# zhupan007/Detection_3D

Measured on AMD Instinct MI355X. Metric: buildings/sec inference, 4c_fpn432, higher is better.
Workload: dtype f32

## Files before the change

### detection_3d_amd/csrc/roi_align.hip

```cpp
#include <algorithm>

#include "d3d_internal.h"

namespace d3d {

struct RoiGeom {
  int b;
  float cw, ch, cz, bh, bw, bz, sh, sw, sz, cosT, sinT;
  int gh, gw, gz;
};
__device__ __forceinline__ RoiGeom roi_geom(const float *r, float spatial_scale, int PH, int PW, int PZ,
                                            int sampling_ratio) {
  RoiGeom g;
  g.b = (int)r[0];
  g.cw = r[1] * spatial_scale;
  g.ch = r[2] * spatial_scale;
  g.cz = r[3] * spatial_scale;
  float rw = r[4] * spatial_scale, rh = r[5] * spatial_scale, rz = r[6] * spatial_scale;
  const float theta = (float)((double)r[7] * 3.14159265358979323846 / 180.0);
  rw = fmaxf(rw, 1.f);
  rh = fmaxf(rh, 1.f);
  rz = fmaxf(rz, 1.f);
  g.bh = rh / (float)PH;
  g.bw = rw / (float)PW;
  g.bz = rz / (float)PZ;
  g.gh = sampling_ratio > 0 ? sampling_ratio : (int)ceilf(rh / PH);
  g.gw = sampling_ratio > 0 ? sampling_ratio : (int)ceilf(rw / PW);
  g.gz = sampling_ratio > 0 ? sampling_ratio : (int)ceilf(rz / PZ);
  g.sh = (float)(-rh / 2.0);
  g.sw = (float)(-rw / 2.0);
  g.sz = (float)(-rz / 2.0);
  g.cosT = (float)cos((double)theta);
  g.sinT = (float)sin((double)theta);
  return g;
}
__device__ __forceinline__ void sample_pos(const RoiGeom &g, int ph, int pw, int pz, int iy, int ix,
                                           int iz, float &y, float &x, float &z) {
  const float yy = g.sh + ph * g.bh + (float)(iy + .5f) * g.bh / (float)g.gh;
  const float xx = g.sw + pw * g.bw + (float)(ix + .5f) * g.bw / (float)g.gw;
  const float zz = g.sz + pz * g.bz + (float)(iz + .5f) * g.bz / (float)g.gz;
  x = xx * g.cosT + yy * g.sinT + g.cw;
  y = yy * g.cosT - xx * g.sinT + g.ch;
  z = zz + g.cz;
}
struct Tri {
  int yl, yh, xl, xh, zl, zh;
  float ly, lx, lz, hy, hx, hz;
};
__device__ __forceinline__ bool tri_setup(float y, float x, float z, int H, int W, int Z, Tri &t) {
  if (y < -1.0 || y > H || x < -1.0 || x > W || z < -1.0) return false;
  if (y <= 0) y = 0;
  if (x <= 0) x = 0;
  if (z <= 0) z = 0;
  t.yl = (int)y;
  t.xl = (int)x;
  t.zl = (int)z;
  if (t.yl >= H - 1) { t.yh = t.yl = H - 1; y = (float)t.yl; } else t.yh = t.yl + 1;
  if (t.xl >= W - 1) { t.xh = t.xl = W - 1; x = (float)t.xl; } else t.xh = t.xl + 1;
  if (t.zl >= Z - 1) { t.zh = t.zl = Z - 1; z = (float)t.zl; } else t.zh = t.zl + 1;
  t.ly = y - t.yl;
  t.lx = x - t.xl;
  t.lz = z - t.zl;
  t.hy = 1. - t.ly;
  t.hx = 1. - t.lx;
  t.hz = 1. - t.lz;
  return true;
}

__global__ __launch_bounds__(256) void k_roi_dense(const float *__restrict__ input, int C, int H,
                                                   int W, int Z, const float *__restrict__ rois,
                                                   long nthreads, float spatial_scale, int PH, int PW,
                                                   int PZ, int sampling_ratio, float *__restrict__ out) {
  long index = (long)blockIdx.x * blockDim.x + threadIdx.x;
  if (index >= nthreads) return;
  const int pz = index % PZ;
  const int pw = (index / PZ) % PW;
  const int ph = (index / PZ / PW) % PH;
  const int c = (index / PZ / PW / PH) % C;
  const int n = index / PZ / PW / PH / C;
  const RoiGeom g = roi_geom(rois + (size_t)n * 8, spatial_scale, PH, PW, PZ, sampling_ratio);
  const float *d = input + ((size_t)g.b * C + c) * H * W * Z;
  const float count = (float)(g.gh * g.gw * g.gz);
  float acc = 0.f;
  for (int iy = 0; iy < g.gh; iy++)
    for (int ix = 0; ix < g.gw; ix++)
      for (int iz = 0; iz < g.gz; iz++) {
        float y, x, z;
        sample_pos(g, ph, pw, pz, iy, ix, iz, y, x, z);
        Tri t;
        if (!tri_setup(y, x, z, H, W, Z, t)) continue;
        const float v1 = d[(t.yl * W + t.xl) * Z + t.zl], v2 = d[(t.yl * W + t.xh) * Z + t.zl];
        const float v3 = d[(t.yh * W + t.xl) * Z + t.zl], v4 = d[(t.yh * W + t.xh) * Z + t.zl];
        const float v5 = d[(t.yl * W + t.xl) * Z + t.zh], v6 = d[(t.yl * W + t.xh) * Z + t.zh];
        const float v7 = d[(t.yh * W + t.xl) * Z + t.zh], v8 = d[(t.yh * W + t.xh) * Z + t.zh];
        const float w1 = t.hy * t.hx * t.hz, w2 = t.hy * t.lx * t.hz, w3 = t.ly * t.hx * t.hz, w4 = t.ly * t.lx * t.hz;
        const float w5 = t.hy * t.hx * t.lz, w6 = t.hy * t.lx * t.lz, w7 = t.ly * t.hx * t.lz, w8 = t.ly * t.lx * t.lz;
        acc += (w1 * v1 + w2 * v2 + w3 * v3 + w4 * v4 + w5 * v5 + w6 * v6 + w7 * v7 + w8 * v8);
      }
  out[index] = acc / count;
}

static constexpr int kRoiG = 4;
static constexpr int kRoiCch = 128;
__device__ __forceinline__ void roi_wave_sync() {
  __builtin_amdgcn_fence(__ATOMIC_RELEASE, "wavefront");
  __builtin_amdgcn_wave_barrier();
  __builtin_amdgcn_fence(__ATOMIC_ACQUIRE, "wavefront");
}
static constexpr int kRoiWaves = 4;
struct RoiLevel {
  const HashEntry *tab;
  const void *feats;
  const int32_t *extent;
  const int32_t *dense;
  int cap, H, W, Z;
  int e0, e1, e2;
  float scale;
};
static constexpr int kRoiMaxLevels = 4;
struct RoiLevels {
  RoiLevel v[kRoiMaxLevels];
};
template <typename T>
__global__ __launch_bounds__(kRoiWaves * 64) __attribute__((amdgpu_waves_per_eu(4, 4))) void k_roi_sparse(
    RoiLevels lv, int C, const float *__restrict__ rois, const int32_t *__restrict__ roi_levels,
    int PH, int PW, int PZ, int sampling_ratio, int layout, T *__restrict__ out) {
  const int n = blockIdx.x, cc = blockIdx.y;
  const int l = roi_levels ? __builtin_amdgcn_readfirstlane(roi_levels[n]) : 0;
  if (l < 0 || l >= kRoiMaxLevels) return;
  RoiLevel L = lv.v[0];
  if (l == 1) L = lv.v[1];
  if (l == 2) L = lv.v[2];
  if (l == 3) L = lv.v[3];
  if (!L.tab) return;
  const HashEntry *__restrict__ tab = L.tab;
  const int32_t *__restrict__ dense = L.dense;
  const T *__restrict__ feats = (const T *)L.feats;
  const int cap = L.cap;
  const float spatial_scale = L.scale;
  int H = L.H, W = L.W, Z = L.Z;
  if (L.extent) {
    H = L.extent[0];
    W = L.extent[1];
    Z = L.extent[2];
  }
  typedef float f32x2 __attribute__((ext_vector_type(2)));
  __shared__ int2 list[kRoiWaves][kRoiG][64];
  const int NB = PH * PW * PZ;
  const int wave = threadIdx.x >> 6, lane = threadIdx.x & 63;
  const RoiGeom g = roi_geom(rois + (size_t)n * 8, spatial_scale, PH, PW, PZ, sampling_ratio);
  const int NS = g.gh * g.gw * g.gz;
  const float count = (float)NS;
  const int c0 = cc * kRoiCch + 2 * lane;
  const bool ok0 = c0 < C, ok1 = c0 + 1 < C;
  const bool pair = ok1 && (C % 2 == 0);
  const size_t n_out = (size_t)n;
  auto load2 = [&](int row) -> f32x2 {
    const T *p = feats + (size_t)row * C + c0;
    f32x2 v = {0.f, 0.f};
    if (pair) {
      if constexpr (sizeof(T) == 4) {
        v = *(const f32x2 *)p;
      } else {
        const unsigned u = *(const unsigned *)p;
        v[0] = __uint_as_float(u << 16);
        v[1] = __uint_as_float(u & 0xffff0000u);
      }
    } else {
      if (ok0) v[0] = ld1(p);
      if (ok1) v[1] = ld1(p + 1);
    }
    return v;
  };
  const int ngroups = (NB + kRoiG - 1) / kRoiG;
  for (int grp = wave; grp < ngroups; grp += kRoiWaves) {
    const int b0 = grp * kRoiG;
    f32x2 acc[kRoiG];
#pragma unroll
    for (int gi = 0; gi < kRoiG; gi++) acc[gi] = {0.f, 0.f};
    for (int s0 = 0; s0 < NS; s0 += 8) {
      const int s = s0 + (lane >> 3), corner = lane & 7;
      const int iz = s % g.gz, ix = (s / g.gz) % g.gw, iy = s / (g.gz * g.gw);
      const int zb = corner >> 2, yb = (corner >> 1) & 1, xb = corner & 1;
      int row[kRoiG];
      float wgt[kRoiG];
      static_assert(kRoiG % 4 == 0, "probe groups of four");
#pragma unroll
      for (int g0 = 0; g0 < kRoiG; g0 += 4) {
        uint64_t key[4];
        bool want[4];
        int r4[4];
#pragma unroll
        for (int j = 0; j < 4; j++) {
          const int bin = b0 + g0 + j;
          wgt[g0 + j] = 0.f;
          key[j] = 0;
          want[j] = false;
          if (s < NS && bin < NB) {
            const int pz = bin % PZ, pw = (bin / PZ) % PW, ph = bin / (PZ * PW);
            float y, x, z;
            sample_pos(g, ph, pw, pz, iy, ix, iz, y, x, z);
            Tri t;
            if (tri_setup(y, x, z, H, W, Z, t)) {
              wgt[g0 + j] = (yb ? t.ly : t.hy) * (xb ? t.lx : t.hx) * (zb ? t.lz : t.hz);
              key[j] = pack_key(g.b, yb ? t.yh : t.yl, xb ? t.xh : t.xl, zb ? t.zh : t.zl);
              want[j] = true;
            }
          }
        }
        if (dense) {
          int v4[4];
#pragma unroll
          for (int j = 0; j < 4; j++) {
            const uint64_t kk = key[j];
            const size_t cell = ((((size_t)(kk >> 48) * L.e0 + (size_t)((kk >> 32) & 0xffff)) * L.e1 +
                                  (size_t)((kk >> 16) & 0xffff)) * L.e2 + (size_t)(kk & 0xffff));
            v4[j] = want[j] ? dense[cell] : 0;
          }
#pragma unroll
          for (int j = 0; j < 4; j++) r4[j] = v4[j] - 1;
        } else {
          hash_find_n<4>(tab, cap, key, want, r4);
        }
#pragma unroll
        for (int j = 0; j < 4; j++) row[g0 + j] = r4[j];
      }
      int cnt[kRoiG];
#pragma unroll
      for (int gi = 0; gi < kRoiG; gi++) {
        unsigned long long m = __ballot(row[gi] >= 0);
        int c = 0;
        while (m) {
          const int rl = __shfl(row[gi], __builtin_ctzll(m), 64);
          const bool mine = row[gi] == rl;
          float w = mine ? wgt[gi] : 0.f;
#pragma unroll
          for (int d = 32; d >= 1; d >>= 1) w += __shfl_xor(w, d, 64);
          if (lane == 0) list[wave][gi][c] = make_int2(rl, __float_as_int(w));
          c++;
          m &= ~__ballot(mine);
        }
        cnt[gi] = c;
      }
      roi_wave_sync();
#pragma unroll
      for (int gi = 0; gi < kRoiG; gi++) {
        const int2 *L = list[wave][gi];
        const int nc = cnt[gi];
        int i = 0;
        for (; i + 8 <= nc; i += 8) {
          int2 e[8];
          f32x2 v[8];
#pragma unroll
          for (int j = 0; j < 8; j++) e[j] = L[i + j];
#pragma unroll
          for (int j = 0; j < 8; j++) v[j] = load2(e[j].x);
#pragma unroll
          for (int j = 0; j < 8; j++) acc[gi] += __int_as_float(e[j].y) * v[j];
        }
        if (i + 4 <= nc) {
          int2 e[4];
          f32x2 v[4];
#pragma unroll
          for (int j = 0; j < 4; j++) e[j] = L[i + j];
#pragma unroll
          for (int j = 0; j < 4; j++) v[j] = load2(e[j].x);
#pragma unroll
          for (int j = 0; j < 4; j++) acc[gi] += __int_as_float(e[j].y) * v[j];
          i += 4;
        }
        if (i + 2 <= nc) {
          const int2 e0 = L[i], e1 = L[i + 1];
          const f32x2 v0 = load2(e0.x), v1 = load2(e1.x);
          acc[gi] += __int_as_float(e0.y) * v0;
          acc[gi] += __int_as_float(e1.y) * v1;
          i += 2;
        }
        if (i < nc) {
          const int2 e0 = L[i];
          acc[gi] += __int_as_float(e0.y) * load2(e0.x);
        }
      }
      roi_wave_sync();
    }
#pragma unroll
    for (int gi = 0; gi < kRoiG; gi++) {
      const int bin = b0 + gi;
      if (bin >= NB) break;
      const f32x2 r = acc[gi] / count;
      if (layout == 0) {
        T *o = out + (n_out * C + c0) * NB + bin;
        if (ok0) st1(o, r[0]);
        if (ok1) st1(o + NB, r[1]);
      } else {
        const int pz = bin % PZ, cell = bin / PZ;
        T *o = out + ((n_out * (size_t)(PH * PW) + cell) * C + c0) * PZ + pz;
        if (ok0) st1(o, r[0]);
        if (ok1) st1(o + PZ, r[1]);
      }
    }
  }
}

__global__ __launch_bounds__(256) void k_roi_dense_bwd(const float *__restrict__ top_diff, int C, int H, int W,
                                                       int Z, const float *__restrict__ rois, long nthreads,
                                                       float spatial_scale, int PH, int PW, int PZ,
                                                       int sampling_ratio, float *__restrict__ bottom_diff) {
  long index = (long)blockIdx.x * blockDim.x + threadIdx.x;
  if (index >= nthreads) return;
  const int pz = index % PZ;
  const int pw = (index / PZ) % PW;
  const int ph = (index / PZ / PW) % PH;
  const int c = (index / PZ / PW / PH) % C;
  const int n = index / PZ / PW / PH / C;
  const RoiGeom g = roi_geom(rois + (size_t)n * 8, spatial_scale, PH, PW, PZ, sampling_ratio);
  float *d = bottom_diff + ((size_t)g.b * C + c) * H * W * Z;
  const float count = (float)(g.gh * g.gw * g.gz);
  const float top = top_diff[index];
  for (int iy = 0; iy < g.gh; iy++)
    for (int ix = 0; ix < g.gw; ix++)
      for (int iz = 0; iz < g.gz; iz++) {
        float y, x, z;
        sample_pos(g, ph, pw, pz, iy, ix, iz, y, x, z);
        Tri t;
        if (z > Z || !tri_setup(y, x, z, H, W, Z, t)) continue;
        const float w[8] = {t.hy * t.hx * t.hz, t.hy * t.lx * t.hz, t.ly * t.hx * t.hz, t.ly * t.lx * t.hz,
                            t.hy * t.hx * t.lz, t.hy * t.lx * t.lz, t.ly * t.hx * t.lz, t.ly * t.lx * t.lz};
#pragma unroll
        for (int q = 0; q < 8; q++) {
          const int yy = (q >> 1) & 1 ? t.yh : t.yl, xx = q & 1 ? t.xh : t.xl, zz = q >> 2 ? t.zh : t.zl;
          atomicAdd(d + ((size_t)yy * W + xx) * Z + zz, top * w[q] / count);
        }
      }
}

static constexpr int kRoiBwdCch = 64;
template <typename TT>
__global__ __launch_bounds__(256) void k_roi_sparse_bwd(
    const HashEntry *__restrict__ tab, int cap, int C, int H, int W, int Z, const float *__restrict__ rois,
    float spatial_scale, int PH, int PW, int PZ, int sampling_ratio, const TT *__restrict__ top_diff,
    float *__restrict__ d_feats) {
  extern __shared__ float tile[];
  const int n = blockIdx.x, cc = blockIdx.y;
  const int NB = PH * PW * PZ, LD = NB + 1;
  const int wave = threadIdx.x >> 6, lane = threadIdx.x & 63;
  const int nch = min(kRoiBwdCch, C - cc * kRoiBwdCch);
  const TT *g0 = top_diff + ((size_t)n * C + (size_t)cc * kRoiBwdCch) * NB;
  for (int idx = threadIdx.x; idx < nch * NB; idx += 256) tile[(idx / NB) * LD + idx % NB] = ld1(g0 + idx);
  __syncthreads();
  const RoiGeom g = roi_geom(rois + (size_t)n * 8, spatial_scale, PH, PW, PZ, sampling_ratio);
  const int NS = g.gh * g.gw * g.gz;
  const float count = (float)NS;
  const int c = cc * kRoiBwdCch + lane;
  const bool cok = c < C;
  for (int bin = wave; bin < NB; bin += 4) {
    const int pz = bin % PZ, pw = (bin / PZ) % PW, ph = bin / (PZ * PW);
    const float top = cok ? tile[lane * LD + bin] : 0.f;
    for (int s0 = 0; s0 < NS; s0 += 8) {
      const int s = s0 + (lane >> 3), corner = lane & 7;
      int row = -1;
      float wgt = 0.f;
      if (s < NS) {
        const int iz = s % g.gz, ix = (s / g.gz) % g.gw, iy = s / (g.gz * g.gw);
        float y, x, z;
        sample_pos(g, ph, pw, pz, iy, ix, iz, y, x, z);
        Tri t;
        if (!(z > Z) && tri_setup(y, x, z, H, W, Z, t)) {
          const int zb = corner >> 2, yb = (corner >> 1) & 1, xb = corner & 1;
          wgt = (yb ? t.ly : t.hy) * (xb ? t.lx : t.hx) * (zb ? t.lz : t.hz);
          row = hash_find(tab, cap, pack_key(g.b, yb ? t.yh : t.yl, xb ? t.xh : t.xl, zb ? t.zh : t.zl));
        }
      }
      unsigned long long m = __ballot(row >= 0);
      while (m) {
        const int rr = __shfl(row, __builtin_ctzll(m), 64);
        const bool mine = row == rr;
        float ww = mine ? wgt : 0.f;
#pragma unroll
        for (int d = 32; d >= 1; d >>= 1) ww += __shfl_xor(ww, d, 64);
        if (cok) atomicAdd(d_feats + (size_t)rr * C + c, top * ww / count);
        m &= ~__ballot(mine);
      }
    }
  }
}

static constexpr int kRoiDetChunk = 64;
static constexpr int kRoiDetCpl = 4;

template <typename TT>
__global__ __launch_bounds__(256) void k_roi_det_transpose(const TT *__restrict__ in, int C, int NB,
                                                           float *__restrict__ out) {
  __shared__ float t[32][33];
  const int n = blockIdx.x, b0 = blockIdx.y * 32, c0 = blockIdx.z * 32;
  const int tx = threadIdx.x & 31, ty = threadIdx.x >> 5;
  const TT *src = in + (size_t)n * C * NB;
  for (int j = ty; j < 32; j += 8) {
    const int c = c0 + j, b = b0 + tx;
    t[j][tx] = (c < C && b < NB) ? ld1(src + (size_t)c * NB + b) : 0.f;
  }
  __syncthreads();
  float *dst = out + (size_t)n * NB * C;
  for (int j = ty; j < 32; j += 8) {
    const int b = b0 + j, c = c0 + tx;
    if (c < C && b < NB) dst[(size_t)b * C + c] = t[tx][j];
  }
}

template <bool WRITE>
__global__ __launch_bounds__(256) void k_roi_det_taps(
    const HashEntry *__restrict__ tab, int cap, int H, int W, int Z, const float *__restrict__ rois,
    float spatial_scale, int PH, int PW, int PZ, int sampling_ratio, int n_rows, int32_t *__restrict__ cnt,
    const int32_t *__restrict__ offs, uint32_t *__restrict__ rec_key, int32_t *__restrict__ rec_val,
    int32_t *__restrict__ rec_src, float *__restrict__ rec_w) {
  const int n = blockIdx.x;
  const int NB = PH * PW * PZ;
  const int wave = threadIdx.x >> 6, lane = threadIdx.x & 63;
  const RoiGeom g = roi_geom(rois + (size_t)n * 8, spatial_scale, PH, PW, PZ, sampling_ratio);
  const int NS = g.gh * g.gw * g.gz;
  const float count = (float)NS;
  for (int bin = wave; bin < NB; bin += 4) {
    const int pz = bin % PZ, pw = (bin / PZ) % PW, ph = bin / (PZ * PW);
    const int src = n * NB + bin;
    int pos = WRITE ? offs[src] : 0;
    for (int s0 = 0; s0 < NS; s0 += 8) {
      const int s = s0 + (lane >> 3), corner = lane & 7;
      int row = -1;
      float wgt = 0.f;
      if (s < NS) {
        const int iz = s % g.gz, ix = (s / g.gz) % g.gw, iy = s / (g.gz * g.gw);
        float y, x, z;
        sample_pos(g, ph, pw, pz, iy, ix, iz, y, x, z);
        Tri t;
        if (!(z > Z) && tri_setup(y, x, z, H, W, Z, t)) {
          const int zb = corner >> 2, yb = (corner >> 1) & 1, xb = corner & 1;
          wgt = (yb ? t.ly : t.hy) * (xb ? t.lx : t.hx) * (zb ? t.lz : t.hz);
          row = hash_find(tab, cap, pack_key(g.b, yb ? t.yh : t.yl, xb ? t.xh : t.xl, zb ? t.zh : t.zl));
          if (row >= n_rows) row = -1;
        }
      }
      unsigned long long m = __ballot(row >= 0);
      while (m) {
        const int rr = __shfl(row, __builtin_ctzll(m), 64);
        const bool mine = row == rr;
        if (WRITE) {
          float ww = mine ? wgt : 0.f;
#pragma unroll
          for (int d = 32; d >= 1; d >>= 1) ww += __shfl_xor(ww, d, 64);
          if (lane == 0) {
            rec_key[pos] = (uint32_t)rr;
            rec_val[pos] = pos;
            rec_src[pos] = src;
            rec_w[pos] = ww / count;
          }
        }
        pos++;
        m &= ~__ballot(mine);
      }
    }
    if (!WRITE && lane == 0) cnt[src] = pos;
  }
}

__global__ __launch_bounds__(256) void k_roi_det_bounds(const uint32_t *__restrict__ skey, int n_max,
                                                        const int32_t *__restrict__ total, int32_t *__restrict__ rbeg,
                                                        int32_t *__restrict__ rend) {
  const int i = blockIdx.x * 256 + threadIdx.x;
  const int n = *total;
  if (i >= n || i >= n_max) return;
  const uint32_t k = skey[i];
  if (i == 0 || skey[i - 1] != k) rbeg[k] = i;
  if (i == n - 1 || skey[i + 1] != k) rend[k] = i + 1;
}

template <typename TO>
__global__ __launch_bounds__(256) void k_roi_det_sum(const uint32_t *__restrict__ skey, const int32_t *__restrict__ sval,
                                                     const int32_t *__restrict__ rec_src, const float *__restrict__ rec_w,
                                                     int n_max, const int32_t *__restrict__ total,
                                                     const int32_t *__restrict__ rbeg, const int32_t *__restrict__ rend,
                                                     const float *__restrict__ topT, int C, float *__restrict__ part,
                                                     TO *__restrict__ d_feats) {
  const int wave = threadIdx.x >> 6, lane = threadIdx.x & 63;
  const int chunk = blockIdx.x * 4 + wave;
  const int a = chunk * kRoiDetChunk;
  const int n = min(*total, n_max);
  if (a >= n) return;
  const int len = min(kRoiDetChunk, n - a);
  int my_key = -1, my_src = 0;
  float my_w = 0.f;
  if (lane < len) {
    my_key = (int)skey[a + lane];
    const int v = sval[a + lane];
    my_src = rec_src[v];
    my_w = rec_w[v];
  }
  for (int cb = 0; cb < C; cb += 64 * kRoiDetCpl) {
    float acc[kRoiDetCpl];
#pragma unroll
    for (int j = 0; j < kRoiDetCpl; j++) acc[j] = 0.f;
    int cur = __shfl(my_key, 0, 64), seg = 0;
    auto flush = [&](int row, int sa, int sb) {
      const bool whole = rbeg[row] == a + sa && rend[row] == a + sb;
      if (whole) {
        TO *dst = d_feats + (size_t)row * C;
#pragma unroll
        for (int j = 0; j < kRoiDetCpl; j++) {
          const int c = cb + lane + 64 * j;
          if (c < C) {
            if constexpr (sizeof(TO) == 4) dst[c] = dst[c] + acc[j];
            else st1(dst + c, acc[j]);
          }
          acc[j] = 0.f;
        }
      } else {
        float *dst = part + ((size_t)chunk * 2 + (sa == 0 ? 0 : 1)) * C;
#pragma unroll
        for (int j = 0; j < kRoiDetCpl; j++) {
          const int c = cb + lane + 64 * j;
          if (c < C) dst[c] = acc[j];
          acc[j] = 0.f;
        }
      }
    };
    for (int p0 = 0; p0 < len; p0 += 4) {
      int key[4], src[4];
      float w[4], v[4][kRoiDetCpl];
#pragma unroll
      for (int q = 0; q < 4; q++) {
        key[q] = __shfl(my_key, p0 + q, 64);
        src[q] = __shfl(my_src, p0 + q, 64);
        w[q] = __shfl(my_w, p0 + q, 64);
      }
#pragma unroll
      for (int q = 0; q < 4; q++)
#pragma unroll
        for (int j = 0; j < kRoiDetCpl; j++) {
          const int c = cb + lane + 64 * j;
          v[q][j] = (p0 + q < len && c < C) ? topT[(size_t)src[q] * C + c] : 0.f;
        }
#pragma unroll
      for (int q = 0; q < 4; q++) {
        if (p0 + q >= len) break;
        if (key[q] != cur) {
          flush(cur, seg, p0 + q);
          cur = key[q];
          seg = p0 + q;
        }
#pragma unroll
        for (int j = 0; j < kRoiDetCpl; j++) acc[j] += w[q] * v[q][j];
      }
    }
    flush(cur, seg, len);
  }
}

template <typename TO>
__global__ __launch_bounds__(256) void k_roi_det_join(const int32_t *__restrict__ rbeg, const int32_t *__restrict__ rend,
                                                      int n_rows, const float *__restrict__ part, int C,
                                                      TO *__restrict__ d_feats) {
  const int row = blockIdx.x * 4 + (threadIdx.x >> 6), lane = threadIdx.x & 63;
  if (row >= n_rows) return;
  const int rb = rbeg[row], re = rend[row];
  if (re <= rb) return;
  const int c0 = rb / kRoiDetChunk, c1 = (re - 1) / kRoiDetChunk;
  if (c0 == c1) return;
  for (int c = lane; c < C; c += 64) {
    float acc = 0.f;
    for (int k = c0; k <= c1; k++) {
      const int slot = (k == c0 && rb != k * kRoiDetChunk) ? 1 : 0;
      acc += part[((size_t)k * 2 + slot) * C + c];
    }
    if constexpr (sizeof(TO) == 4) d_feats[(size_t)row * C + c] += acc;
    else st1(d_feats + (size_t)row * C + c, acc);
  }
}

__global__ __launch_bounds__(256) void k_roi_f32_to_bf16(const float *__restrict__ in, long n,
                                                         unsigned short *__restrict__ out) {
  const long i = ((long)blockIdx.x * 256 + threadIdx.x) * 4;
  if (i + 4 <= n)
    store4(out + i, load4<float>(in + i));
  else
    for (long j = i; j < n; j++) st1(out + j, in[j]);
}

struct RoiDetLayout {
  size_t cnt, offs, total, scan, rkey, rval, rsrc, rw, skey, sval, sort, rbeg, rend, topT, part, bytes;
  size_t scan_bytes, sort_bytes;
  long n_max, n_src, n_chunks;
  int bits;
};
static bool roi_det_layout(int K, int C, int ph, int pw, int pz, int sampling_ratio, int n_rows, RoiDetLayout &L) {
  if (K < 0 || C <= 0 || ph <= 0 || pw <= 0 || pz <= 0 || sampling_ratio <= 0 || n_rows < 0) return false;
  const long NB = (long)ph * pw * pz, NS = (long)sampling_ratio * sampling_ratio * sampling_ratio;
  L.n_src = (long)K * NB;
  L.n_max = L.n_src * NS * 8;
  if (L.n_max >= (1L << 31) - kRoiDetChunk) return false;
  L.n_chunks = (L.n_max + kRoiDetChunk - 1) / kRoiDetChunk;
  L.bits = 1;
  while (L.bits < 31 && (1L << L.bits) < (long)n_rows) L.bits++;
  size_t o = 0;
  auto take = [&](size_t bytes) {
    const size_t at = o;
    o = (o + bytes + 255) & ~size_t(255);
    return at;
  };
  L.cnt = take(4 * L.n_src);
  L.offs = take(4 * L.n_src);
  L.total = take(4);
  L.scan_bytes = 4 * ((L.n_src + 2047) / 2048 + 1) + 256;
  L.scan = take(L.scan_bytes);
  L.rkey = take(4 * L.n_max);
  L.rval = take(4 * L.n_max);
  L.rsrc = take(4 * L.n_max);
  L.rw = take(4 * L.n_max);
  L.skey = take(4 * L.n_max);
  L.sval = take(4 * L.n_max);
  L.sort_bytes = sort_scratch_bytes((int)std::max(L.n_max, 1L), L.bits);
  L.sort = take(L.sort_bytes);
  L.rbeg = take(4 * (size_t)n_rows);
  L.rend = take(4 * (size_t)n_rows);
  L.topT = take(4 * (size_t)L.n_src * C);
  L.part = take(4 * (size_t)L.n_chunks * 2 * C);
  L.bytes = o + 256;
  return true;
}

static constexpr int kRoiFormFields = 13;
static thread_local int t_roi_last_form[kRoiFormFields] = {};
enum RoiFamily { kRoiFamDense = 1, kRoiFamSparse = 2, kRoiFamDenseBwd = 3, kRoiFamSparseBwd = 4, kRoiFamDet = 5 };
static void roi_record(int family, size_t type_bytes, int lookup, int extent, dim3 grid, int block, int levels, long cvt = 0,
                       long n_max = 0, long n_chunks = 0, int bits = 0) {
  const int f[kRoiFormFields] = {family, type_bytes == 4 ? 1 : 2, lookup, extent, (int)grid.x, (int)grid.y, (int)grid.z,
                                 block, levels, (int)cvt, (int)n_max, (int)n_chunks, bits};
  std::copy(f, f + kRoiFormFields, t_roi_last_form);
}
static void roi_record_sparse(const RoiLevels &lv, size_t type_bytes, dim3 grid) {
  int lookup = 0, extent = 0, levels = 0;
  for (int l = 0; l < kRoiMaxLevels; l++) {
    if (!lv.v[l].tab) continue;
    levels++;
    lookup |= lv.v[l].dense ? 2 : 1;
    extent |= lv.v[l].extent ? 2 : 1;
  }
  roi_record(kRoiFamSparse, type_bytes, lookup, extent, grid, kRoiWaves * 64, levels);
}

}

using namespace d3d;

struct RoiPrepScales {
  float v[8];
};
__global__ __launch_bounds__(256) void k_roi_prepare(const float *__restrict__ boxes, int n, float voxel_scale,
                                                     RoiPrepScales scales, int n_levels, float inv_canonical,
                                                     float *__restrict__ rois, int32_t *__restrict__ levels,
                                                     const int32_t *__restrict__ batch_ids,
                                                     const int32_t *__restrict__ count) {
  const int i = blockIdx.x * blockDim.x + threadIdx.x;
  if (i >= n) return;
  if (count && i >= *count) {
    float *r = rois + (size_t)i * 8;
#pragma unroll
    for (int j = 0; j < 8; j++) r[j] = 0.f;
    if (levels) levels[i] = -1;
    return;
  }
  float b[7];
#pragma unroll
  for (int j = 0; j < 7; j++) b[j] = boxes[(size_t)i * 7 + j];
#pragma unroll
  for (int j = 0; j < 6; j++) b[j] *= voxel_scale;
  const float kHalfPi = (float)(3.14159265358979323846 * 0.5), kPi = (float)3.14159265358979323846;
  const float kInvPi = 1.f / kPi, kDeg = (float)(180.0 / 3.14159265358979323846);
  float yaw = b[6] + kHalfPi;
  yaw = yaw - floorf(yaw * kInvPi + 0.f) * kPi;
  float *r = rois + (size_t)i * 8;
  r[0] = batch_ids ? (float)batch_ids[i] : 0.f;
  r[1] = b[1];
  r[2] = b[0];
  r[3] = b[2] + b[5] * 0.5f;
  r[4] = b[3];
  r[5] = b[4];
  r[6] = b[5];
  r[7] = yaw * kDeg;
  if (levels) {
    const float rate = sqrtf(fmaxf(b[3], b[4])) * inv_canonical;
    int best = 0;
    float bd = fabsf(scales.v[0] - rate);
    for (int l = 1; l < n_levels; l++) {
      const float d = fabsf(scales.v[l] - rate);
      if (d < bd) {
        bd = d;
        best = l;
      }
    }
    levels[i] = best;
  }
}

extern "C" {

int d3d_roi_prepare(const float *boxes_metric, int n, float voxel_scale, const float *scales_host, int n_levels,
                    float canonical_size, const int32_t *batch_ids, float *rois, int32_t *levels, void *stream) {
  return d3d_roi_prepare_counted(boxes_metric, n, nullptr, voxel_scale, scales_host, n_levels, canonical_size, batch_ids,
                                 rois, levels, stream);
}

int d3d_roi_prepare_counted(const float *boxes_metric, int n, const int32_t *count_dev, float voxel_scale,
                            const float *scales_host, int n_levels, float canonical_size, const int32_t *batch_ids,
                            float *rois, int32_t *levels, void *stream) {
  hipStream_t s = (hipStream_t)stream;
  D3D_REQUIRE(n >= 0 && n_levels >= 0 && n_levels <= 8, "roi_prepare: bad arguments (at most 8 levels)");
  if (n == 0) return D3D_OK;
  D3D_REQUIRE(boxes_metric && rois && (n_levels == 0 || scales_host), "roi_prepare: null pointer");
  RoiPrepScales sc = {};
  for (int l = 0; l < n_levels; l++) sc.v[l] = scales_host[l];
  hipLaunchKernelGGL(k_roi_prepare, dim3((unsigned)((n + 255) / 256)), dim3(256), 0, s, boxes_metric, n, voxel_scale, sc,
                     n_levels, 1.f / canonical_size, rois, n_levels > 1 ? levels : nullptr, batch_ids, count_dev);
  D3D_LAUNCH_CHECK();
  return D3D_OK;
}

int d3d_roi_align_rotated_3d_forward(const float *input, int B, int C, int H, int W, int Z,
                                     const float *rois, int K, float spatial_scale, int ph, int pw,
                                     int pz, int sampling_ratio, float *out, void *stream) {
  hipStream_t s = (hipStream_t)stream;
  D3D_REQUIRE(B > 0 && C > 0 && H > 0 && W > 0 && Z > 0 && K >= 0 && ph > 0 && pw > 0 && pz > 0, "roi_align: bad shape");
  if (K == 0) return D3D_OK;
  D3D_REQUIRE(input && rois && out, "roi_align: null pointer");
  long nthreads = (long)K * C * ph * pw * pz;
  hipLaunchKernelGGL(k_roi_dense, dim3((unsigned)((nthreads + 255) / 256)), dim3(256), 0, s, input, C, H, W, Z, rois, nthreads, spatial_scale, ph, pw, pz, sampling_ratio, out);
  D3D_LAUNCH_CHECK();
  roi_record(kRoiFamDense, 4, 0, 0, dim3((unsigned)((nthreads + 255) / 256)), 256, 0);
  return D3D_OK;
}

static int roi_level_of(d3d_meta *m, const int *size, const void *feats, const int *crop, float spatial_scale,
                        hipStream_t s, RoiLevel *lv) {
  std::map<Size3, Grid>::iterator it;
  bool have_grid;
  {
    D3D_LOCK(m);
    it = m->grids.find(Size3{size[0], size[1], size[2]});
    have_grid = it != m->grids.end();
  }
  if (!have_grid) {
    set_error("roi_align_sparse: no grid of spatial size [%d,%d,%d]", size[0], size[1], size[2]);
    return D3D_ERR_STATE;
  }
  Grid &g = it->second;
  const int32_t *extent = nullptr;
  if (!crop) {
    int rc = grid_extent(m, g, s);
    if (rc) return rc;
    extent = g.extent;
  }
  *lv = {g.tab, feats, extent, crop ? nullptr : g.dense, g.cap, crop ? crop[0] : 0, crop ? crop[1] : 0, crop ? crop[2] : 0,
         g.hext[0], g.hext[1], g.hext[2], spatial_scale};
  return D3D_OK;
}

}

template <typename T>
static int roi_sparse_forward(d3d_meta *m, const int *size, const T *feats, int C, const int *crop, const float *rois, int K,
                              float spatial_scale, int ph, int pw, int pz, int sampling_ratio, const int *roi_levels,
                              int level, int layout, T *out, void *stream) {
  hipStream_t s = (hipStream_t)stream;
  D3D_REQUIRE(m && size && C > 0 && K >= 0 && ph > 0 && pw > 0 && pz > 0, "roi_align_sparse: bad arguments");
  D3D_REQUIRE(!roi_levels || (level >= 0 && level < kRoiMaxLevels), "roi_align_sparse: level %d (< %d)", level, kRoiMaxLevels);
  D3D_REQUIRE(sizeof(T) == 4 || ((uintptr_t)feats & 3) == 0, "roi_align_sparse: bf16 rows not 4-byte aligned");
  RoiLevels lv = {};
  if (int rc = roi_level_of(m, size, feats, crop, spatial_scale, s, &lv.v[roi_levels ? level : 0])) return rc;
  if (K == 0) return D3D_OK;
  D3D_REQUIRE(feats && rois && out, "roi_align_sparse: null pointer");
  D3D_REQUIRE(layout == 0 || layout == 1, "roi_align_sparse: layout must be 0 ([K,C,ph,pw,pz]) or 1 ([K,ph,pw,C,pz])");
  hipLaunchKernelGGL(k_roi_sparse<T>, dim3(K, (C + kRoiCch - 1) / kRoiCch), dim3(kRoiWaves * 64), 0, s, lv, C, rois,
                     roi_levels, ph, pw, pz, sampling_ratio, layout, out);
  D3D_LAUNCH_CHECK();
  roi_record_sparse(lv, sizeof(T), dim3(K, (C + kRoiCch - 1) / kRoiCch));
  return D3D_OK;
}

template <typename T>
static int roi_sparse_forward_levels(d3d_meta *m, int n_levels, const int *sizes_host, const T *const *feats_host, int C,
                                     const float *scales_host, const float *rois, int K, int ph, int pw, int pz,
                                     int sampling_ratio, const int *roi_levels, int layout, T *out, void *stream) {
  hipStream_t s = (hipStream_t)stream;
  D3D_REQUIRE(m && sizes_host && feats_host && scales_host && n_levels >= 1 && n_levels <= kRoiMaxLevels,
              "roi_align_sparse_levels: 1..%d levels", kRoiMaxLevels);
  D3D_REQUIRE(C > 0 && K >= 0 && ph > 0 && pw > 0 && pz > 0 && (roi_levels || n_levels == 1),
              "roi_align_sparse_levels: bad arguments");
  D3D_REQUIRE(layout == 0 || layout == 1, "roi_align_sparse: layout must be 0 ([K,C,ph,pw,pz]) or 1 ([K,ph,pw,C,pz])");
  RoiLevels lv = {};
  for (int l = 0; l < n_levels; l++) {
    D3D_REQUIRE(feats_host[l], "roi_align_sparse_levels: null feature pointer of level %d", l);
    D3D_REQUIRE(sizeof(T) == 4 || ((uintptr_t)feats_host[l] & 3) == 0, "roi_align_sparse_levels: bf16 rows not 4-byte aligned");
    if (int rc = roi_level_of(m, sizes_host + 3 * l, feats_host[l], nullptr, scales_host[l], s, &lv.v[l])) return rc;
  }
  if (K == 0) return D3D_OK;
  D3D_REQUIRE(rois && out, "roi_align_sparse_levels: null pointer");
  hipLaunchKernelGGL(k_roi_sparse<T>, dim3(K, (C + kRoiCch - 1) / kRoiCch), dim3(kRoiWaves * 64), 0, s, lv, C, rois,
                     roi_levels, ph, pw, pz, sampling_ratio, layout, out);
  D3D_LAUNCH_CHECK();
  roi_record_sparse(lv, sizeof(T), dim3(K, (C + kRoiCch - 1) / kRoiCch));
  return D3D_OK;
}

extern "C" {

int d3d_roi_align_rotated_3d_sparse_forward(d3d_meta *m, const int *size, const float *feats, int C,
                                            const int *crop, const float *rois, int K,
                                            float spatial_scale, int ph, int pw, int pz,
                                            int sampling_ratio, const int *roi_levels, int level, int layout,
                                            float *out, void *stream) {
  return roi_sparse_forward<float>(m, size, feats, C, crop, rois, K, spatial_scale, ph, pw, pz, sampling_ratio, roi_levels,
                                   level, layout, out, stream);
}

int d3d_roi_align_rotated_3d_sparse_forward_bf16(d3d_meta *m, const int *size, const void *feats, int C, const int *crop,
                                                 const float *rois, int K, float spatial_scale, int ph, int pw, int pz,
                                                 int sampling_ratio, const int *roi_levels, int level, int layout,
                                                 void *out, void *stream) {
  return roi_sparse_forward<unsigned short>(m, size, (const unsigned short *)feats, C, crop, rois, K, spatial_scale, ph,
                                            pw, pz, sampling_ratio, roi_levels, level, layout, (unsigned short *)out,
                                            stream);
}

int d3d_roi_align_rotated_3d_sparse_forward_levels(d3d_meta *m, int n_levels, const int *sizes_host,
                                                   const float *const *feats_host, int C, const float *scales_host,
                                                   const float *rois, int K, int ph, int pw, int pz, int sampling_ratio,
                                                   const int *roi_levels, int layout, float *out, void *stream) {
  return roi_sparse_forward_levels<float>(m, n_levels, sizes_host, feats_host, C, scales_host, rois, K, ph, pw, pz,
                                          sampling_ratio, roi_levels, layout, out, stream);
}

int d3d_roi_align_rotated_3d_sparse_forward_levels_bf16(d3d_meta *m, int n_levels, const int *sizes_host,
                                                        const void *const *feats_host, int C, const float *scales_host,
                                                        const float *rois, int K, int ph, int pw, int pz,
                                                        int sampling_ratio, const int *roi_levels, int layout, void *out,
                                                        void *stream) {
  return roi_sparse_forward_levels<unsigned short>(m, n_levels, sizes_host, (const unsigned short *const *)feats_host, C,
                                                   scales_host, rois, K, ph, pw, pz, sampling_ratio, roi_levels, layout,
                                                   (unsigned short *)out, stream);
}

int d3d_roi_align_rotated_3d_backward(const float *top_diff, int B, int C, int H, int W, int Z,
                                      const float *rois, int K, float spatial_scale, int ph, int pw, int pz,
                                      int sampling_ratio, float *bottom_diff, void *stream) {
  hipStream_t s = (hipStream_t)stream;
  D3D_REQUIRE(B > 0 && C > 0 && H > 0 && W > 0 && Z > 0 && K >= 0 && ph > 0 && pw > 0 && pz > 0 && bottom_diff,
              "roi_align_backward: bad arguments");
  D3D_HIP_CHECK(hipMemsetAsync(bottom_diff, 0, sizeof(float) * (size_t)B * C * H * W * Z, s));
  if (K == 0) return D3D_OK;
  D3D_REQUIRE(top_diff && rois, "roi_align_backward: null pointer");
  long nthreads = (long)K * C * ph * pw * pz;
  hipLaunchKernelGGL(k_roi_dense_bwd, dim3((unsigned)((nthreads + 255) / 256)), dim3(256), 0, s, top_diff, C, H, W, Z,
                     rois, nthreads, spatial_scale, ph, pw, pz, sampling_ratio, bottom_diff);
  D3D_LAUNCH_CHECK();
  roi_record(kRoiFamDenseBwd, 4, 0, 0, dim3((unsigned)((nthreads + 255) / 256)), 256, 0);
  return D3D_OK;
}

static int roi_grid_of(d3d_meta *m, const int *size, const char *what, const Grid **out) {
  std::map<Size3, Grid>::iterator it;
  bool have_grid;
  {
    D3D_LOCK(m);
    it = m->grids.find(Size3{size[0], size[1], size[2]});
    have_grid = it != m->grids.end();
  }
  if (!have_grid) {
    set_error("%s: no grid of spatial size [%d,%d,%d]", what, size[0], size[1], size[2]);
    return D3D_ERR_STATE;
  }
  *out = &it->second;
  return D3D_OK;
}

int d3d_roi_align_rotated_3d_sparse_backward(d3d_meta *m, const int *size, const float *top_diff, int C,
                                             const int *crop, const float *rois, int K, float spatial_scale,
                                             int ph, int pw, int pz, int sampling_ratio, float *d_feats,
                                             void *stream) {
  hipStream_t s = (hipStream_t)stream;
  D3D_REQUIRE(m && size && crop && C > 0 && K >= 0 && ph > 0 && pw > 0 && pz > 0, "roi_align_sparse_backward: bad arguments");
  const Grid *gp;
  if (int rc = roi_grid_of(m, size, "roi_align_sparse_backward", &gp)) return rc;
  if (K == 0) return D3D_OK;
  D3D_REQUIRE(top_diff && rois && d_feats, "roi_align_sparse_backward: null pointer");
  const Grid &g = *gp;
  const int NB = ph * pw * pz;
  size_t lds = (size_t)kRoiBwdCch * (NB + 1) * sizeof(float);
  D3D_REQUIRE(lds <= 64 * 1024, "roi_align_sparse_backward: pooled volume %d too large", NB);
  hipLaunchKernelGGL(k_roi_sparse_bwd<float>, dim3(K, (C + kRoiBwdCch - 1) / kRoiBwdCch), dim3(256), lds, s, g.tab, g.cap,
                     C, crop[0], crop[1], crop[2], rois, spatial_scale, ph, pw, pz, sampling_ratio, top_diff, d_feats);
  D3D_LAUNCH_CHECK();
  roi_record(kRoiFamSparseBwd, 4, 1, 1, dim3(K, (C + kRoiBwdCch - 1) / kRoiBwdCch), 256, 1);
  return D3D_OK;
}

size_t d3d_roi_align_rotated_3d_sparse_backward_bf16_scratch_bytes(int C, int n_rows) {
  if (C <= 0 || n_rows < 0) return 0;
  return (size_t)n_rows * C * sizeof(float) + 256;
}

int d3d_roi_align_rotated_3d_sparse_backward_bf16(d3d_meta *m, const int *size, const void *top_diff, int C,
                                                  const int *crop, const float *rois, int K, float spatial_scale, int ph,
                                                  int pw, int pz, int sampling_ratio, void *d_feats, int n_rows,
                                                  void *scratch, size_t scratch_bytes, void *stream) {
  hipStream_t s = (hipStream_t)stream;
  D3D_REQUIRE(m && size && crop && C > 0 && K >= 0 && ph > 0 && pw > 0 && pz > 0 && n_rows >= 0,
              "roi_align_sparse_backward_bf16: bad arguments");
  const int NB = ph * pw * pz;
  const size_t lds = (size_t)kRoiBwdCch * (NB + 1) * sizeof(float);
  D3D_REQUIRE(lds <= 64 * 1024, "roi_align_sparse_backward_bf16: pooled volume %d too large", NB);
  const size_t need = d3d_roi_align_rotated_3d_sparse_backward_bf16_scratch_bytes(C, n_rows);
  D3D_REQUIRE(scratch_bytes >= need, "roi_align_sparse_backward_bf16: scratch %zu < %zu bytes", scratch_bytes, need);
  const Grid *gp;
  if (int rc = roi_grid_of(m, size, "roi_align_sparse_backward_bf16", &gp)) return rc;
  D3D_REQUIRE(n_rows == gp->n, "roi_align_sparse_backward_bf16: n_rows %d != %d active sites", n_rows, gp->n);
  if (n_rows == 0) return D3D_OK;
  D3D_REQUIRE(d_feats && scratch && (K == 0 || (top_diff && rois)), "roi_align_sparse_backward_bf16: null pointer");
  D3D_REQUIRE(((uintptr_t)d_feats & 7) == 0, "roi_align_sparse_backward_bf16: d_feats not 8-byte aligned");
  float *acc = (float *)(((uintptr_t)scratch + 255) & ~(uintptr_t)255);
  const long total = (long)n_rows * C;
  D3D_HIP_CHECK(hipMemsetAsync(acc, 0, sizeof(float) * (size_t)total, s));
  if (K > 0) {
    const Grid &g = *gp;
    hipLaunchKernelGGL(k_roi_sparse_bwd<unsigned short>, dim3(K, (C + kRoiBwdCch - 1) / kRoiBwdCch), dim3(256), lds, s,
                       g.tab, g.cap, C, crop[0], crop[1], crop[2], rois, spatial_scale, ph, pw, pz, sampling_ratio,
                       (const unsigned short *)top_diff, acc);
  }
  hipLaunchKernelGGL(k_roi_f32_to_bf16, dim3((unsigned)((total + 1023) / 1024)), dim3(256), 0, s, acc, total,
                     (unsigned short *)d_feats);
  D3D_LAUNCH_CHECK();
  roi_record(kRoiFamSparseBwd, 2, 1, 1, K > 0 ? dim3(K, (C + kRoiBwdCch - 1) / kRoiBwdCch) : dim3(0, 0, 0), 256, 1,
             (total + 1023) / 1024);
  return D3D_OK;
}

size_t d3d_roi_align_rotated_3d_sparse_backward_deterministic_scratch_bytes(int K, int C, int ph, int pw, int pz,
                                                                           int sampling_ratio, int n_rows) {
  RoiDetLayout L;
  return roi_det_layout(K, C, ph, pw, pz, sampling_ratio, n_rows, L) ? L.bytes : 0;
}

size_t d3d_roi_align_rotated_3d_sparse_backward_deterministic_bf16_scratch_bytes(int K, int C, int ph, int pw, int pz,
                                                                                int sampling_ratio, int n_rows) {
  return d3d_roi_align_rotated_3d_sparse_backward_deterministic_scratch_bytes(K, C, ph, pw, pz, sampling_ratio, n_rows);
}

}

template <typename TT, typename TO>
static int roi_det_run(const Grid &g, const int *crop, const TT *top_diff, int C, const float *rois, int K,
                       float spatial_scale, int ph, int pw, int pz, int sampling_ratio, TO *d_feats, int n_rows,
                       const RoiDetLayout &L, void *scratch, hipStream_t s) {
  char *base = (char *)(((uintptr_t)scratch + 255) & ~(uintptr_t)255);
  int32_t *cnt = (int32_t *)(base + L.cnt), *offs = (int32_t *)(base + L.offs), *total = (int32_t *)(base + L.total);
  uint32_t *rkey = (uint32_t *)(base + L.rkey), *skey = (uint32_t *)(base + L.skey);
  int32_t *rval = (int32_t *)(base + L.rval), *sval = (int32_t *)(base + L.sval), *rsrc = (int32_t *)(base + L.rsrc);
  float *rw = (float *)(base + L.rw), *topT = (float *)(base + L.topT), *part = (float *)(base + L.part);
  int32_t *rbeg = (int32_t *)(base + L.rbeg), *rend = (int32_t *)(base + L.rend);
  const int NB = ph * pw * pz;
  hipLaunchKernelGGL(k_roi_det_transpose<TT>, dim3(K, (NB + 31) / 32, (C + 31) / 32), dim3(256), 0, s, top_diff, C, NB,
                     topT);
  hipLaunchKernelGGL((k_roi_det_taps<false>), dim3(K), dim3(256), 0, s, g.tab, g.cap, crop[0], crop[1], crop[2], rois,
                     spatial_scale, ph, pw, pz, sampling_ratio, n_rows, cnt, nullptr, nullptr, nullptr, nullptr, nullptr);
  D3D_LAUNCH_CHECK();
  Arena scan_arena;
  scan_arena.base = base + L.scan;
  scan_arena.cap = L.scan_bytes;
  if (int rc = scan_exclusive_i32(cnt, offs, (int)L.n_src, total, scan_arena, s)) return rc;
  hipLaunchKernelGGL((k_roi_det_taps<true>), dim3(K), dim3(256), 0, s, g.tab, g.cap, crop[0], crop[1], crop[2], rois,
                     spatial_scale, ph, pw, pz, sampling_ratio, n_rows, nullptr, offs, rkey, rval, rsrc, rw);
  D3D_LAUNCH_CHECK();
  Arena sort_arena;
  sort_arena.base = base + L.sort;
  sort_arena.cap = L.sort_bytes;
  if (int rc = sort_pairs_u32(rkey, skey, rval, sval, (int)L.n_max, L.bits, sort_arena, s, false, total)) return rc;
  D3D_HIP_CHECK(hipMemsetAsync(rbeg, 0, 4 * (size_t)n_rows, s));
  D3D_HIP_CHECK(hipMemsetAsync(rend, 0, 4 * (size_t)n_rows, s));
  hipLaunchKernelGGL(k_roi_det_bounds, dim3((unsigned)((L.n_max + 255) / 256)), dim3(256), 0, s, skey, (int)L.n_max,
                     total, rbeg, rend);
  hipLaunchKernelGGL(k_roi_det_sum<TO>, dim3((unsigned)((L.n_chunks + 3) / 4)), dim3(256), 0, s, skey, sval, rsrc, rw,
                     (int)L.n_max, total, rbeg, rend, topT, C, part, d_feats);
  hipLaunchKernelGGL(k_roi_det_join<TO>, dim3((unsigned)((n_rows + 3) / 4)), dim3(256), 0, s, rbeg, rend, n_rows, part, C,
                     d_feats);
  D3D_LAUNCH_CHECK();
  roi_record(kRoiFamDet, sizeof(TO), 1, 1, dim3((unsigned)((L.n_chunks + 3) / 4)), 256, 1, 0, L.n_max, L.n_chunks, L.bits);
  return D3D_OK;
}

extern "C" {

int d3d_roi_last_form(int *out, int n) {
  for (int i = 0; out && i < n && i < kRoiFormFields; i++) out[i] = t_roi_last_form[i];
  std::fill(t_roi_last_form, t_roi_last_form + kRoiFormFields, 0);
  return kRoiFormFields;
}

int d3d_roi_align_rotated_3d_sparse_backward_deterministic(d3d_meta *m, const int *size, const float *top_diff, int C,
                                                           const int *crop, const float *rois, int K,
                                                           float spatial_scale, int ph, int pw, int pz,
                                                           int sampling_ratio, float *d_feats, int n_rows,
                                                           void *scratch, size_t scratch_bytes, void *stream) {
  hipStream_t s = (hipStream_t)stream;
  D3D_REQUIRE(m && size && crop && C > 0 && K >= 0 && ph > 0 && pw > 0 && pz > 0 && n_rows >= 0,
              "roi_align_sparse_backward_deterministic: bad arguments");
  D3D_REQUIRE(sampling_ratio > 0,
              "roi_align_sparse_backward_deterministic: sampling_ratio %d (adaptive sampling has no record bound before "
              "the launch)", sampling_ratio);
  const Grid *gp;
  if (int rc = roi_grid_of(m, size, "roi_align_sparse_backward_deterministic", &gp)) return rc;
  if (K == 0 || n_rows == 0) return D3D_OK;
  D3D_REQUIRE(top_diff && rois && d_feats && scratch, "roi_align_sparse_backward_deterministic: null pointer");
  RoiDetLayout L;
  D3D_REQUIRE(roi_det_layout(K, C, ph, pw, pz, sampling_ratio, n_rows, L),
              "roi_align_sparse_backward_deterministic: %d RoIs x %d bins x %d samples is too many records", K,
              ph * pw * pz, sampling_ratio * sampling_ratio * sampling_ratio);
  D3D_REQUIRE(scratch_bytes >= L.bytes, "roi_align_sparse_backward_deterministic: scratch %zu < %zu bytes", scratch_bytes,
              L.bytes);
  return roi_det_run<float, float>(*gp, crop, top_diff, C, rois, K, spatial_scale, ph, pw, pz, sampling_ratio, d_feats,
                                   n_rows, L, scratch, s);
}

int d3d_roi_align_rotated_3d_sparse_backward_deterministic_bf16(d3d_meta *m, const int *size, const void *top_diff, int C,
                                                                const int *crop, const float *rois, int K,
                                                                float spatial_scale, int ph, int pw, int pz,
                                                                int sampling_ratio, void *d_feats, int n_rows,
                                                                void *scratch, size_t scratch_bytes, void *stream) {
  hipStream_t s = (hipStream_t)stream;
  D3D_REQUIRE(m && size && crop && C > 0 && K >= 0 && ph > 0 && pw > 0 && pz > 0 && n_rows >= 0,
              "roi_align_sparse_backward_deterministic_bf16: bad arguments");
  D3D_REQUIRE(sampling_ratio > 0,
              "roi_align_sparse_backward_deterministic_bf16: sampling_ratio %d (adaptive sampling has no record bound "
              "before the launch)", sampling_ratio);
  RoiDetLayout L;
  D3D_REQUIRE(roi_det_layout(K, C, ph, pw, pz, sampling_ratio, n_rows, L),
              "roi_align_sparse_backward_deterministic_bf16: %d RoIs x %d bins x %d samples is too many records", K,
              ph * pw * pz, sampling_ratio * sampling_ratio * sampling_ratio);
  D3D_REQUIRE(K == 0 || scratch_bytes >= L.bytes, "roi_align_sparse_backward_deterministic_bf16: scratch %zu < %zu bytes",
              scratch_bytes, L.bytes);
  const Grid *gp;
  if (int rc = roi_grid_of(m, size, "roi_align_sparse_backward_deterministic_bf16", &gp)) return rc;
  D3D_REQUIRE(n_rows == gp->n, "roi_align_sparse_backward_deterministic_bf16: n_rows %d != %d active sites", n_rows,
              gp->n);
  if (n_rows == 0) return D3D_OK;
  D3D_REQUIRE(d_feats && (K == 0 || (top_diff && rois && scratch)),
              "roi_align_sparse_backward_deterministic_bf16: null pointer");
  D3D_HIP_CHECK(hipMemsetAsync(d_feats, 0, sizeof(unsigned short) * (size_t)n_rows * C, s));
  if (K == 0) return D3D_OK;
  return roi_det_run<unsigned short, unsigned short>(*gp, crop, (const unsigned short *)top_diff, C, rois, K, spatial_scale,
                                                     ph, pw, pz, sampling_ratio, (unsigned short *)d_feats, n_rows, L,
                                                     scratch, s);
}

}
```

Before: 214.5.

## Batch ROI cell weight reductions with DPP/permlane and vectorize bin stores

Replaces the per-unique-cell 6-step shfl_xor weight reduction with a flattened cell list whose weights are reduced eight cells at a time. The reduction packs four cells per pass using permlane32/16 swaps and DPP row ops, and uses readlane instead of shfl for broadcasting row ids. It also adds a wide vectorized store path that writes four PZ bins per channel in one instruction when layout==1 and PZ==4. The aim is to cut cross-lane shuffle latency and scattered scalar stores, at the cost of more complex lane-index bookkeeping and reliance on gfx950-specific permlane swap intrinsics.

```diff
diff --git a/detection_3d_amd/csrc/roi_align.hip b/detection_3d_amd/csrc/roi_align.hip
--- a/detection_3d_amd/csrc/roi_align.hip
+++ b/detection_3d_amd/csrc/roi_align.hip
@@ -108,6 +108,28 @@
   __builtin_amdgcn_fence(__ATOMIC_ACQUIRE, "wavefront");
 }
 static constexpr int kRoiWaves = 4;
+static constexpr int kRoiB = 8;
+
+template <int CTRL>
+__device__ __forceinline__ float roi_dpp(float v) {
+  return __int_as_float(__builtin_amdgcn_update_dpp(0, __float_as_int(v), CTRL, 0xf, 0xf, true));
+}
+__device__ __forceinline__ float roi_pack32(float a, float b) {
+  const auto r = __builtin_amdgcn_permlane32_swap(__float_as_uint(a), __float_as_uint(b), false, false);
+  return __uint_as_float(r[0]) + __uint_as_float(r[1]);
+}
+__device__ __forceinline__ float roi_pack16(float p, float q) {
+  const auto r = __builtin_amdgcn_permlane16_swap(__float_as_uint(p), __float_as_uint(q), false, false);
+  return __uint_as_float(r[0]) + __uint_as_float(r[1]);
+}
+__device__ __forceinline__ float roi_cells4_sum(float a, float b, float c, float d) {
+  float v = roi_pack16(roi_pack32(a, b), roi_pack32(c, d));
+  v += roi_dpp<0x128>(v);
+  v += roi_dpp<0x1B>(roi_dpp<0x141>(v));
+  v += roi_dpp<0x4E>(v);
+  v += roi_dpp<0xB1>(v);
+  return v;
+}
 struct RoiLevel {
   const HashEntry *tab;
   const void *feats;
@@ -145,7 +167,7 @@
     Z = L.extent[2];
   }
   typedef float f32x2 __attribute__((ext_vector_type(2)));
-  __shared__ int2 list[kRoiWaves][kRoiG][64];
+  __shared__ int2 list[kRoiWaves][kRoiG * 64];
   const int NB = PH * PW * PZ;
   const int wave = threadIdx.x >> 6, lane = threadIdx.x & 63;
   const RoiGeom g = roi_geom(rois + (size_t)n * 8, spatial_scale, PH, PW, PZ, sampling_ratio);
@@ -172,6 +194,9 @@
     }
     return v;
   };
+  static_assert(kRoiG == 4, "the wide store writes four bins per channel");
+  const bool wide = layout == 1 && PZ == kRoiG && (cc + 1) * kRoiCch <= C &&
+                    ((uintptr_t)out & (kRoiG * sizeof(T) - 1)) == 0;
   const int ngroups = (NB + kRoiG - 1) / kRoiG;
   for (int grp = wave; grp < ngroups; grp += kRoiWaves) {
     const int b0 = grp * kRoiG;
@@ -225,27 +250,51 @@
 #pragma unroll
         for (int j = 0; j < 4; j++) row[g0 + j] = r4[j];
       }
-      int cnt[kRoiG];
+      int2 *lst = list[wave];
+      int cnt[kRoiG], base[kRoiG], flat[kRoiG];
+      int total = 0;
 #pragma unroll
       for (int gi = 0; gi < kRoiG; gi++) {
         unsigned long long m = __ballot(row[gi] >= 0);
-        int c = 0;
+        int c = 0, fl = -1, cellrow = 0;
         while (m) {
-          const int rl = __shfl(row[gi], __builtin_ctzll(m), 64);
+          const int rl = __builtin_amdgcn_readlane(row[gi], __builtin_ctzll(m));
           const bool mine = row[gi] == rl;
-          float w = mine ? wgt[gi] : 0.f;
-#pragma unroll
-          for (int d = 32; d >= 1; d >>= 1) w += __shfl_xor(w, d, 64);
-          if (lane == 0) list[wave][gi][c] = make_int2(rl, __float_as_int(w));
+          fl = mine ? total + c : fl;
+          cellrow = lane == c ? rl : cellrow;
           c++;
           m &= ~__ballot(mine);
         }
+        if (lane < c) lst[total + lane].x = cellrow;
+        flat[gi] = fl;
+        base[gi] = total;
         cnt[gi] = c;
+        total += c;
+      }
+      for (int f0 = 0; f0 < total; f0 += kRoiB) {
+        float sm[kRoiB];
+#pragma unroll
+        for (int k = 0; k < kRoiB; k++) sm[k] = 0.f;
+#pragma unroll
+        for (int gi = 0; gi < kRoiG; gi++) {
+          if (base[gi] < f0 + kRoiB && base[gi] + cnt[gi] > f0) {
+            const int e = flat[gi] - f0;
+#pragma unroll
+            for (int k = 0; k < kRoiB; k++) sm[k] = e == k ? wgt[gi] : sm[k];
+          }
+        }
+#pragma unroll
+        for (int h = 0; h < kRoiB; h += 4) {
+          const float w = roi_cells4_sum(sm[h], sm[h + 1], sm[h + 2], sm[h + 3]);
+          const int q = lane >> 4;
+          const int f = f0 + h + (((q & 1) << 1) | (q >> 1));
+          if ((lane & 15) == 0 && f < total) lst[f].y = __float_as_int(w);
+        }
       }
       roi_wave_sync();
 #pragma unroll
       for (int gi = 0; gi < kRoiG; gi++) {
-        const int2 *L = list[wave][gi];
+        const int2 *L = lst + base[gi];
         const int nc = cnt[gi];
         int i = 0;
         for (; i + 8 <= nc; i += 8) {
@@ -282,6 +331,25 @@
         }
       }
       roi_wave_sync();
+    }
+    if (wide) {
+      f32x2 r[kRoiG];
+#pragma unroll
+      for (int gi = 0; gi < kRoiG; gi++) r[gi] = acc[gi] / count;
+      T *o = out + ((n_out * (size_t)(PH * PW) + grp) * C + c0) * kRoiG;
+#pragma unroll
+      for (int ch = 0; ch < 2; ch++) {
+        if constexpr (sizeof(T) == 4) {
+          const d3d_f32x4 v = {r[0][ch], r[1][ch], r[2][ch], r[3][ch]};
+          *(d3d_f32x4 *)(o + ch * kRoiG) = v;
+        } else {
+          unsigned short h[kRoiG];
+#pragma unroll
+          for (int gi = 0; gi < kRoiG; gi++) st1(&h[gi], r[gi][ch]);
+          *(uint2 *)(o + ch * kRoiG) = make_uint2(h[0] | (unsigned)h[1] << 16, h[2] | (unsigned)h[3] << 16);
+        }
+      }
+      continue;
     }
 #pragma unroll
     for (int gi = 0; gi < kRoiG; gi++) {
```

New measurement: 221.2 (median of 6 runs). 1.03x the previous value.
